# rcallahan/smalt

Measured on AMD Instinct MI355X. Metric: mapped reads/sec (1Mx150bp vs 3Gbp ref), higher is better.
Workload: dtype f16

## Files before the change

### smalt_amd/csrc/smaltgpu.cpp

```cpp
#include <hip/hip_runtime.h>
#include <math.h>
#include <stdarg.h>
#include <stdio.h>
#include <stdlib.h>
#include <string.h>
#include <mutex>
#include <string>
#include <thread>
#include <vector>
#include "../../include/smaltgpu.h"
#include "smg_dump.hpp"
#include "smg_indexfile.hpp"
#include "smg_indexbuild.h"
#include "smg_fasta.hpp"
#include "smg_kernels.h"

using namespace smg;

static thread_local std::string g_err;
static int fail(int code, const char *fmt, ...) {
  char buf[512];
  va_list ap;
  va_start(ap, fmt);
  vsnprintf(buf, sizeof(buf), fmt, ap);
// ... 284 lines not shown
  }
  return ix->packed_host.data();
}

extern "C" int smaltgpu_index_info(const smaltgpu_index *ix, smaltgpu_index_desc *o) {
  if (!ix || !o) return fail(SMALTGPU_EARG, "null argument");
  memset(o, 0, sizeof(*o));
  o->k = ix->d.k; o->s = ix->d.s; o->typ = ix->d.typ; o->nbits_key = ix->d.nbits_key; o->nbits_lo = ix->d.nbits_lo;
  o->npos = ix->d.npos; o->nwords = ix->d.nwords; o->idx = ix->d.idx; o->pos = ix->d.pos; o->wordidx = ix->d.wordidx;
  o->posidx = ix->d.posidx; o->nseq = ix->d.nseq; o->sop = ix->sop.data(); o->packed = ix->d.packed; o->on_device = 1;
  return SMALTGPU_OK;
}

extern "C" void smaltgpu_params_default(smaltgpu_params *p, const smaltgpu_index *ix) {
  memset(p, 0, sizeof(*p));
  p->ktuple_maxhit = 10000;
  p->min_cover = 0;
  p->min_swatscor = ix->d.k + ix->d.s - 1;
  p->min_swatscor_below_max = 0;
  p->min_basqval = 0;
  p->target_depth = 512; p->max_depth = 2048;
  p->rmapflg = SMALTGPU_FLG_BEST | (ix->d.nseq < 512 ? SMALTGPU_FLG_SEQBYSEQ : 0);
  p->match = 1; p->mismatch = -2; p->gap_init = -4; p->gap_ext = -3;
}

enum { T_ENCODE = 0, T_SEED, T_HITS, T_CANDS, T_SW_FULL, T_SW_SCALAR, T_REPLAY, T_ALIGN, T_NUM };
static const char *const kTimerNames[T_NUM] = {"encode", "seed", "hits", "cands", "sw_full", "sw_scalar", "replay", "align"};
extern "C" const char *smaltgpu_timer_name(int i) { return (i >= 0 && i < T_NUM) ? kTimerNames[i] : nullptr; }

struct smaltgpu_mapper {
  const smaltgpu_index *ix = nullptr;
  int device = 0;
  hipStream_t stream = nullptr;
  uint32_t max_reads = 0, max_len = 0, qmax = 0;
  uint64_t max_bases = 0;
  uint8_t *d_bases = nullptr, *d_quals = nullptr, *d_codes = nullptr, *d_codes_rc = nullptr;
  uint64_t *d_off = nullptr;
  uint32_t *d_ids = nullptr;
  uint32_t hits_W = 0, hits_wg = 0;
  HitRun *b_hitrun = nullptr;
  Batch b;
  enum : size_t { CT_LINE = 128, CT_RC = 0, CT_RES = 1 * CT_LINE, CT_DSTR = 2 * CT_LINE, CT_ERR = 3 * CT_LINE, CT_NEXT = 4 * CT_LINE ,
                  CT_ALIGN_RETRY = 9 * CT_LINE, CT_CANDS_RETRY = 10 * CT_LINE, CT_HITS = 11 * CT_LINE, CT_HITS_CURSOR = 12 * CT_LINE, CT_STRIP_CURSOR = 13 * CT_LINE,
                  CT_WORK = 14 * CT_LINE , CT_BYTES = 16 * CT_LINE };
  uint8_t *d_counters = nullptr;
  double *d_logtab = nullptr; uint32_t logtab_n = 0;
  uint8_t *seed_scr = nullptr; size_t seed_bytes = 0; uint32_t seed_slots = 0;
  uint8_t *cand_scr = nullptr; size_t cand_bytes = 0; uint32_t cand_slots = 0;
  CandGeom cg2; uint8_t *cand_scr2 = nullptr; size_t cand_bytes2 = 0; uint32_t cand_slots2 = 0;
  CandGeom cg;
  uint8_t *cand_scr_dbg = nullptr; uint32_t cand_dbg_reads = 0;
  int *sw_rows = nullptr; uint32_t sw_rowlen = 0, sw_threads = 0;
  void *strip_bnd = nullptr; uint8_t *strip_win = nullptr; uint32_t strip_grid = 0;
  uint8_t *align_scr = nullptr; size_t align_bytes = 0; uint32_t align_slots = 0;
  uint8_t *align_scr2 = nullptr; size_t align_bytes2 = 0; uint32_t align_slots2 = 0; uint64_t dircap2 = 0;
  uint32_t wincap = 0, rescap_slot = 0, dstrcap_slot = 0; uint64_t dircap = 0;
  uint32_t rescap_slot2 = 0, dstrcap_slot2 = 0;
  template <class T> struct Pinned {
    T *p = nullptr; size_t cap = 0;
    int ensure(size_t n) {
      if (n <= cap) return 0;
      size_t c = cap ? cap : 1024;
      while (c < n) c += c / 2 + 1;
      T *q = nullptr;
      if (hipHostMalloc((void **)&q, c * sizeof(T), hipHostMallocDefault) != hipSuccess) return -1;
      if (p) (void)hipHostFree(p);
      p = q; cap = c;
      return 0;
    }
    void release() { if (p) (void)hipHostFree(p); p = nullptr; cap = 0; }
    T *data() { return p; }
    T &operator[](size_t i) { return p[i]; }
  };
  Pinned<ReadStat> h_stat;
  Pinned<Result> h_res;
  Pinned<uint8_t> h_dstr;
  hipEvent_t ev_fetch = nullptr;
  uint32_t fetch_n = 0; uint64_t fetch_nres = 0; bool fetch_open = false, pool_overflow = false;
  std::vector<smaltgpu_result> fin_res; std::vector<uint8_t> fin_dstr; std::vector<smaltgpu_readstat> fin_stat; std::vector<uint64_t> fin_off;
  std::vector<uint64_t> h_res_off;
  std::vector<smaltgpu_result> o_res;
  std::vector<smaltgpu_readstat> o_stat;
  std::vector<uint64_t> h_off;
  uint32_t last_n = 0;
  MapPar last_par;
  bool have_host_off = false;
  int debug = 0;
  struct DevBuf {
    void *p = nullptr; size_t cap = 0;
    int ensure(size_t n) { if (n <= cap) return 0; if (p) (void)hipFree(p); p = nullptr; cap = 0; size_t c = n + n / 2 + 256; if (hipMalloc(&p, c) != hipSuccess) return -1; cap = c; return 0; }
    void release() { if (p) (void)hipFree(p); p = nullptr; cap = 0; }
  };
  DevBuf cx_ivoff, cx_iv, cx_minsw, cx_prevmax, cx_fineidx, cx_finepos, cx_fineoff, cx_alloclen, cx_seedrange;
  int host_threads = 1;
  bool history = false;
  uint32_t hist_longest = 0;
  std::vector<uint32_t> h_alloclen;
  std::vector<uint32_t> h_ivoff, h_fineoff;
  std::vector<HitInfoHdr> h_hi;
  bool last_fine = false;
  uint64_t remap_batches = 0;
  hipEvent_t ev[T_NUM + 1] = {nullptr};
  double ms[T_NUM] = {0};
  unsigned long long work[WK_NWORK] = {0};
};

// ... 123 lines not shown
      const size_t fixed = 64  + seqb + (size_t)5 * m->cg.tab * 4 + 64 + 15 + 256 ;
      uint32_t w = fixed + 23 * 256 < 20480 ? (uint32_t)((20480 - fixed) / 23) & ~7u : 256u;
      if (w < (uint32_t)CANDS_LDS_HITS / 2) w = CANDS_LDS_HITS;
      const char *e = getenv("SMALTGPU_CANDS_LDS_HITS");
      m->cg.lds_hits = e ? (uint32_t)atoi(e) : w;
    }
    if (m->cg.lds_hits < 256) m->cg.lds_hits = 256;
    if (m->cg.lds_hits > 2048) m->cg.lds_hits = 2048;
    m->cg.slot_bytes = m->cand_bytes = cand_slot_bytes(m->cg, m->qmax, d.s);
    memset(&m->cg2, 0, sizeof(m->cg2));
    auto geom_for = [&](uint64_t hs) { CandGeom g = m->cg; g.hcap_strand = (uint32_t)hs; g.hcap = (uint32_t)(2 * hs); g.segcap = (uint32_t)hs; g.candcap = (uint32_t)(2 * hs);
                                       g.slot_bytes = cand_slot_bytes(g, m->qmax, d.s); return g; };
    const CandGeom full = m->cg;
    if (m->cand_bytes > (64ull << 20)) {
      uint64_t hs = next_pow2((uint64_t)24 * m->qmax);
      if (const char *e = getenv("SMALTGPU_CANDS_HCAP")) { const long v = atol(e); if (v >= 1024) hs = next_pow2((uint64_t)v); }
      if (hs < m->cg.hcap_strand) { m->cg = geom_for(hs); m->cand_bytes = m->cg.slot_bytes; }
    } else if (const char *e = getenv("SMALTGPU_CANDS_HCAP")) {
      const long v = atol(e);
      if (v >= 1024 && next_pow2((uint64_t)v) < m->cg.hcap_strand) { m->cg = geom_for(next_pow2((uint64_t)v)); m->cand_bytes = m->cg.slot_bytes; }
    }
    {
      uint64_t hw = next_pow2((uint64_t)m->cg.ngrp * alloc);
      if (hw < full.hcap_strand) hw = full.hcap_strand;
      if (hw < (2ull << 20)) hw = 2ull << 20;
      while (hw > full.hcap_strand && (hw > (1ull << 30) || geom_for(hw).slot_bytes > (4ull << 30))) hw >>= 1;
      if (hw > m->cg.hcap_strand) {
        m->cg2 = geom_for(hw); m->cg2.pass = 2; m->cand_bytes2 = m->cg2.slot_bytes;
        m->cg.pass = 1;
        uint64_t n2 = (opt_budget ? ((uint64_t)opt_budget << 30) / 4 : (8ull << 30)) / m->cand_bytes2;
        if (n2 > 8) n2 = 8;
        if (n2 < 1) n2 = 1;
        if (n2 > max_batch_reads) n2 = max_batch_reads;
        m->cand_slots2 = (uint32_t)n2;
        DA(m->cand_scr2, m->cand_bytes2 * m->cand_slots2);
      }
    }
    uint64_t budget = 64ull << 30;
    if (opt_budget) budget = (uint64_t)opt_budget << 30;
    if (const char *e = getenv("SMALTGPU_SLOT_BUDGET_GB")) { const long g = atol(e); if (g > 0) budget = (uint64_t)g << 30; }
    uint64_t slots = budget / m->cand_bytes;
    if (slots > 2048) slots = 2048;
    if (slots < 64) slots = 64;
    if (slots > max_batch_reads) slots = max_batch_reads;
    m->cand_slots = (uint32_t)slots;
    DA(m->cand_scr, m->cand_bytes * m->cand_slots);
  }
  m->sw_rowlen = m->qmax + 8; m->sw_threads = 16384;
  DA(m->sw_rows, (size_t)m->sw_threads * 2 * m->sw_rowlen);
  {
    m->wincap = 4 * m->qmax + 1024;
    m->strip_grid = 5120;
    if (const char *e = getenv("SMALTGPU_STRIP_GRID")) { const long v = atol(e); if (v >= 64 && v <= 16384) m->strip_grid = (uint32_t)v; }
    if ((uint64_t)m->strip_grid * m->wincap * 18 > (8ull << 30)) m->strip_grid = (uint32_t)((8ull << 30) / ((uint64_t)m->wincap * 18));
    if (!rv) rv = dalloc((uint8_t **)&m->strip_bnd, (size_t)m->strip_grid * 2 * m->wincap * 8);
    DA(m->strip_win, (size_t)m->strip_grid * m->wincap * 2);
    m->dircap = (uint64_t)(m->qmax + 64) * (m->wincap + 8);
    m->rescap_slot = 512; m->dstrcap_slot = 512 * (m->qmax / 4 + 48);
    m->rescap_slot2 = 2 * MAXIMUM_DEPTH; m->dstrcap_slot2 = m->rescap_slot2 * (m->qmax / 4 + 48);
    m->dircap2 = m->dircap;
    if (m->dircap > (4ull << 20)) {
      m->dircap2 = m->dircap;
      m->dircap = m->dircap / 16 > (4ull << 20) ? m->dircap / 16 : (4ull << 20);
      if (const char *e = getenv("SMALTGPU_ALIGN_DIRCAP")) { const long v = atol(e); if (v >= 4096 && (uint64_t)v < m->dircap2) m->dircap = (uint64_t)v; }
    }
    m->align_bytes2 = align_scratch_bytes(m->qmax, m->wincap, m->dircap2, m->rescap_slot2, m->dstrcap_slot2);
    m->align_slots2 = max_batch_reads < 16 ? max_batch_reads : 16;
    DA(m->align_scr2, m->align_bytes2 * m->align_slots2);
    m->align_bytes = align_scratch_bytes(m->qmax, m->wincap, m->dircap, m->rescap_slot, m->dstrcap_slot);
    uint64_t budget = 8ull << 30;
    if (m->align_bytes * 512 > budget) budget = m->align_bytes * 512;
    if (budget > (48ull << 30)) budget = 48ull << 30;
    if (opt_budget && ((uint64_t)opt_budget << 30) < budget) budget = (uint64_t)opt_budget << 30;
    if (const char *e = getenv("SMALTGPU_SLOT_BUDGET_GB")) { const uint64_t g = (uint64_t)atol(e) << 30; if (g > 0 && g < budget) budget = g; }
    uint64_t slots = budget / m->align_bytes;
    if (slots > 8192) slots = 8192;
    if (slots < 16) slots = 16;
    if (slots > max_batch_reads) slots = max_batch_reads;
    m->align_slots = (uint32_t)slots;
    DA(m->align_scr, m->align_bytes * m->align_slots);
  }
#undef DA
  if (rv) { smaltgpu_mapper_free(m); return rv; }
  *out = m;
  return SMALTGPU_OK;
}

extern "C" void smaltgpu_mapper_free(smaltgpu_mapper *m) {
  if (!m) return;
  (void)hipSetDevice(m->device);
  void *ps[] = {m->d_bases, m->d_quals, m->d_codes, m->d_codes_rc, m->d_off, m->d_ids, m->b.hi, m->b.seeds, m->b.qmask, m->b.ch, m->b.ctl,
                m->b.stat, m->b.align_retry, m->b.cands_retry, m->d_logtab, m->b.hitpool, m->b_hitrun, m->b.rcpool, m->b.long_list, m->b.strip_list, m->strip_bnd, m->strip_win, m->b.respool, m->b.dstrpool, m->d_counters, m->seed_scr, m->cand_scr, m->cand_scr2, m->cand_scr_dbg,
                m->sw_rows, m->align_scr, m->align_scr2};
  for (void *p : ps) if (p) (void)hipFree(p);
  m->h_stat.release(); m->h_res.release(); m->h_dstr.release();
  m->cx_ivoff.release(); m->cx_iv.release(); m->cx_minsw.release(); m->cx_prevmax.release(); m->cx_fineidx.release(); m->cx_finepos.release(); m->cx_fineoff.release(); m->cx_alloclen.release(); m->cx_seedrange.release();
  if (m->ev_fetch) (void)hipEventDestroy(m->ev_fetch);
  for (int i = 0; i <= T_NUM; i++) if (m->ev[i]) (void)hipEventDestroy(m->ev[i]);
  if (m->stream) (void)hipStreamDestroy(m->stream);
  delete m;
}

extern "C" int smaltgpu_set_debug(smaltgpu_mapper *m, int level) {
  if (!m) return fail(SMALTGPU_EARG, "null mapper");
  m->debug = level;
  return SMALTGPU_OK;
// ... 23 lines not shown
                        const smaltgpu_params *par, const CtxDev *cx = nullptr, bool seed_only = false) {
  Batch &b = m->b;
  const DevIndex &d = m->ix->d;
  MapPar p = to_par(par);
  b.iv_off = cx ? cx->iv_off : nullptr; b.iv = cx ? cx->iv : nullptr; b.min_sw = cx ? cx->min_sw : nullptr; b.prevmax = cx ? cx->prevmax : nullptr;
  b.fine_idx = cx ? cx->fine_idx : nullptr; b.fine_pos = cx ? cx->fine_pos : nullptr; b.fine_off = cx ? cx->fine_off : nullptr;
  b.alloc_len = cx ? cx->alloc_len : nullptr;
  b.seed_range = cx ? cx->seed_range : nullptr;
  b.totals_only = seed_only ? 1u : 0u;
  b.raw_results = cx ? cx->raw : 0u;
  if (b.fine_idx) p.flags |= FLG_NOSHRTINFO;
  m->last_fine = b.fine_idx != nullptr;
  m->last_par = p; m->last_n = n;
  b.nreads = n; b.codes = m->d_codes; b.codes_rc = m->d_codes_rc; b.qual = d_quals; b.read_off = d_off;
  hipStream_t s = m->stream;
  HIPCHK(hipMemsetAsync(m->d_counters, 0, smaltgpu_mapper::CT_BYTES, s));
  int rv = 0;
  const bool seqbyseq = (p.flags & FLG_SEQBYSEQ) != 0;
  const uint32_t ngrp = seqbyseq ? (uint32_t)d.nseq : 1u;
  uint8_t *cscr = m->cand_scr;
  uint32_t cslots = m->cand_slots;
  int slot_per_read = 0;
  CandGeom cgeom = m->cg;
  const bool two_pass = m->cand_scr2 != nullptr && !m->debug;
  const size_t cbytes_dbg = m->cand_bytes;
  if (m->debug) {
    if (n > 2048) return fail(SMALTGPU_EARG, "debug batches are limited to 2048 reads");
    if (m->cand_dbg_reads < n) {
      if (m->cand_scr_dbg) (void)hipFree(m->cand_scr_dbg);
      m->cand_scr_dbg = nullptr;
      HIPCHK(hipMalloc((void **)&m->cand_scr_dbg, cbytes_dbg * n));
      m->cand_dbg_reads = n;
    }
    cscr = m->cand_scr_dbg; cslots = n; slot_per_read = 1;
  }
  HIPCHK(hipEventRecord(m->ev[T_ENCODE], s));
  rv = launch_encode(s, d_bases, d_off, n, m->d_codes, m->d_codes_rc);
  if (!rv && b.fine_idx) rv = launch_fine_index(s, b, d);
  HIPCHK(hipEventRecord(m->ev[T_SEED], s));
  if (!rv) rv = launch_seed(s, b, d, p, m->seed_scr, m->seed_bytes, m->seed_slots);
  HIPCHK(hipEventRecord(m->ev[T_HITS], s));
  const bool split_hits = m->hits_W && m->b_hitrun && !b.iv_off && !seed_only;
  b.hitrun = split_hits ? m->b_hitrun : nullptr;
  if (!rv && split_hits) rv = launch_hits(s, b, d, p, m->hits_W, m->cg.tab, m->hits_wg);
  HIPCHK(hipEventRecord(m->ev[T_CANDS], s));
  if (seed_only) {
    for (int i = T_CANDS + 1; i <= T_NUM; i++) HIPCHK(hipEventRecord(m->ev[i], s));
    if (rv) return fail(SMALTGPU_ENODEV, "kernel launch failed: %s", hipGetErrorString((hipError_t)rv));
    return SMALTGPU_OK;
  }
  { CandGeom g = cgeom; g.ngrp = ngrp; g.debug = slot_per_read; if (!two_pass) g.pass = 0; if (!rv) rv = launch_cands(s, b, d, p, cscr, cslots, g); }
  if (two_pass) { CandGeom g = m->cg2; g.ngrp = ngrp; g.debug = 0; g.pass = 2; if (!rv) rv = launch_cands(s, b, d, p, m->cand_scr2, m->cand_slots2, g); }
  HIPCHK(hipEventRecord(m->ev[T_SW_FULL], s));
  if (!rv) rv = launch_sw_full(s, b, d, p, m->max_len, b.rccap, 8192);
  HIPCHK(hipEventRecord(m->ev[T_SW_SCALAR], s));
  if (!rv) rv = launch_sw_strip(s, b, d, p, m->strip_bnd, m->strip_win, m->wincap, m->strip_grid);
  if (!rv) rv = launch_sw_scalar(s, b, d, p, m->sw_rows, m->sw_rowlen, m->sw_threads, m->max_len);
  HIPCHK(hipEventRecord(m->ev[T_REPLAY], s));
  if (!rv) rv = launch_replay(s, b, d, p);
  HIPCHK(hipEventRecord(m->ev[T_ALIGN], s));
  CplxPar cplx;
  cplx.logtab = m->d_logtab; cplx.nlog = m->logtab_n; cplx.pad = 0;
  cplx.lambda = (p.flags & FLG_CMPLXW) ? cplx_lambda(p.match, p.mismatch) : 0.0;
  if (!rv) rv = launch_align(s, b, d, p, m->align_scr, m->align_bytes, m->align_slots, m->wincap, m->dircap, m->rescap_slot, m->dstrcap_slot, 1, &cplx);
  if (!rv) rv = launch_align(s, b, d, p, m->align_scr2, m->align_bytes2, m->align_slots2, m->wincap, m->dircap2, m->rescap_slot2, m->dstrcap_slot2, 2, &cplx);
  HIPCHK(hipEventRecord(m->ev[T_NUM], s));
  if (rv) return fail(SMALTGPU_ENODEV, "kernel launch failed: %s", hipGetErrorString((hipError_t)rv));
  return SMALTGPU_OK;
}

extern "C" int smaltgpu_synchronize(smaltgpu_mapper *m) {
  if (!m) return fail(SMALTGPU_EARG, "null mapper");
  HIPCHK(hipStreamSynchronize(m->stream));
  return SMALTGPU_OK;
}

extern "C" int smaltgpu_map_batch_device(smaltgpu_mapper *m, const uint8_t *d_bases, const uint8_t *d_quals, const uint64_t *d_read_off,
                                          uint32_t nreads, uint64_t total_bases, const smaltgpu_params *par) {
  if (!m || !d_bases || !d_read_off || !par) return fail(SMALTGPU_EARG, "null argument");
  if (nreads > m->max_reads || total_bases > m->max_bases) return fail(SMALTGPU_EARG, "batch exceeds the mapper's capacity");
  int rv = check_par(m, par);
  if (rv) return rv;
  HIPCHK(hipSetDevice(m->device));
  m->have_host_off = false;
  return run_pipeline(m, d_bases, d_quals, d_read_off, nreads, par);
}

extern "C" int smaltgpu_fetch_begin(smaltgpu_mapper *m) {
  if (!m) return fail(SMALTGPU_EARG, "null argument");
  HIPCHK(hipSetDevice(m->device));
  const uint32_t n = m->last_n;
  uint8_t ctr[smaltgpu_mapper::CT_BYTES];
  if (!m->ev_fetch) HIPCHK(hipEventCreate(&m->ev_fetch));
  if (m->h_stat.ensure(n ? n : 1)) return fail(SMALTGPU_ENOMEM, "pinned host memory");
  HIPCHK(hipMemcpyAsync(ctr, m->d_counters, smaltgpu_mapper::CT_BYTES, hipMemcpyDeviceToHost, m->stream));
  HIPCHK(hipStreamSynchronize(m->stream));
  const uint32_t rc_count = *(uint32_t *)(ctr + smaltgpu_mapper::CT_RC);
  const uint64_t nres = *(unsigned long long *)(ctr + smaltgpu_mapper::CT_RES), ndstr = *(unsigned long long *)(ctr + smaltgpu_mapper::CT_DSTR);
  memcpy(m->work, ctr + smaltgpu_mapper::CT_WORK, sizeof(m->work));
  for (int i = 0; i < T_NUM; i++) { float f = 0; (void)hipEventElapsedTime(&f, m->ev[i], m->ev[i + 1]); m->ms[i] = f; }
  m->fetch_open = false;
  m->pool_overflow = rc_count > m->b.rccap || nres > m->b.rescap || ndstr > m->b.dstrcap;
  const uint64_t nres_c = nres < m->b.rescap ? nres : m->b.rescap, ndstr_c = ndstr < m->b.dstrcap ? ndstr : m->b.dstrcap;
  if (m->h_res.ensure(nres_c ? nres_c : 1) || m->h_dstr.ensure(ndstr_c ? ndstr_c : 1)) return fail(SMALTGPU_ENOMEM, "pinned host memory");
  if (n) HIPCHK(hipMemcpyAsync(m->h_stat.data(), m->b.stat, (size_t)n * sizeof(ReadStat), hipMemcpyDeviceToHost, m->stream));
  if (nres_c) HIPCHK(hipMemcpyAsync(m->h_res.data(), m->b.respool, nres_c * sizeof(Result), hipMemcpyDeviceToHost, m->stream));
  if (ndstr_c) HIPCHK(hipMemcpyAsync(m->h_dstr.data(), m->b.dstrpool, ndstr_c, hipMemcpyDeviceToHost, m->stream));
// ... 485 lines not shown
```

### smalt_amd/csrc/smg_kernels.hip

```cpp
#include <hip/hip_runtime.h>
#include <cstdlib>
#include "smg_kernels.h"
#include "smg_stages.hpp"

namespace smg {

__device__ inline uint8_t code_of(uint8_t c) {
  c &= 0xDF;
  return c == 'A' ? 0 : c == 'C' ? 1 : c == 'G' ? 2 : (c == 'T' || c == 'U') ? 3 : 5;
}

__global__ void __launch_bounds__(64) k_encode(const uint8_t *bases, const uint64_t *off, uint32_t n, uint8_t *codes, uint8_t *codes_rc) {
  for (uint32_t r = blockIdx.x; r < n; r += gridDim.x) {
    const uint64_t o = off[r];
    const uint32_t len = (uint32_t)(off[r + 1] - o);
    for (uint32_t i = threadIdx.x; i < len; i += 64) {
      uint8_t c = code_of(bases[o + i]);
      codes[o + i] = c;
      codes_rc[o + len - 1 - i] = (c & 4) ? c : (uint8_t)(3 - c);
    }
  }
}

__global__ void __launch_bounds__(64) k_gather_reads(uint8_t *dst_bases, uint8_t *dst_quals, const uint64_t *dst_off, uint32_t n, const uint32_t *ids,
// ... 394 lines not shown
#pragma unroll
    for (int c0 = 0; c0 < C; c0 += SW16_BLK) {
      hf2 t3[SW16_BLK];
      const hf2 last_old = H[(c0 + SW16_BLK - 1 < C) ? c0 + SW16_BLK - 1 : C - 1];
#pragma unroll
      for (int u = 0; u < SW16_BLK; u++) {
        const int cc = c0 + u;
        if (cc < C) {
          const hf2 w = __builtin_bit_cast(hf2, __builtin_amdgcn_perm(rr.y, rr.x, sel[cc]));
          const hf2 dg = u == 0 ? carry : H[cc - 1];
          t3[u] = dg + w;
        }
      }
#pragma unroll
      for (int u = 0; u < SW16_BLK; u++) {
        const int cc = c0 + u;
        if (cc < C) {
          const hf2 hh = hf_max3(t3[u], E[cc], F);
          H[cc] = hh;
          const hf2 tt = hh + ngi;
          E[cc] = hf_max3(E[cc] + nge, tt, zero);
          F = hf_max3(F + nge, tt, zero);
        }
      }
#pragma unroll
      for (int u = 0; u < SW16_BLK; u += 2) {
        const int cc = c0 + u;
        if (cc + 1 < C && u + 1 < SW16_BLK) best = hf_max3(best, H[cc], H[cc + 1]);
        else if (cc < C) best = __builtin_elementwise_maximum(best, H[cc]);
      }
      carry = last_old;
    }
  }
  for (int o = G / 2; o > 0; o >>= 1)
    best = __builtin_elementwise_maximum(best, __builtin_bit_cast(hf2, (uint32_t)__shfl_xor((int)__builtin_bit_cast(uint32_t, best), o)));
  return (uint32_t)(int)(float)best.x | ((uint32_t)(int)(float)best.y << 16);
}

__device__ inline void sw16_rowtab(uint32_t *rowtab, const Sw16Par &sp) {
  if (threadIdx.x < 8) rowtab[threadIdx.x] = threadIdx.x < 4 ? sp.mm4 + (sp.dlt << (8 * threadIdx.x)) : sp.n4;
}
__device__ inline void sw16_rowtab2(uint2 *rowtab2, const Sw16Par &sp) {
  const uint32_t a = threadIdx.x & 7u, bq = threadIdx.x >> 3;
  if (sp.fp) {
    const uint32_t x4 = sp.hi_mismatch * 0x01010101u;
    rowtab2[threadIdx.x] = make_uint2(a < 4 ? (x4 & ~(0xffu << (8 * a))) | (sp.hi_match << (8 * a)) : 0u,
                                      bq < 4 ? (x4 & ~(0xffu << (8 * bq))) | (sp.hi_match << (8 * bq)) : 0u);
    return;
  }
  rowtab2[threadIdx.x] = make_uint2(a < 4 ? sp.mm4 + (sp.dlt << (8 * a)) : sp.n4, bq < 4 ? sp.mm4 + (sp.dlt << (8 * bq)) : sp.n4);
}
enum : uint32_t { SW16_NPAIR = 5u | (5u << 3) };

template <int G, int C, int WMAX>
__global__ void __launch_bounds__(64) k_sw_full16(Batch b, DevIndex ix, MapPar p, uint32_t ntask_cap) {
  const unsigned long long nlong = WMAX > SW_SHORT_WMAX ? b.work[WK_LONG_TASKS] : 0;
  if (WMAX > SW_SHORT_WMAX && nlong == 0) return;
  const uint32_t *list = (WMAX > SW_SHORT_WMAX && b.long_list && nlong <= b.long_cap) ? b.long_list : nullptr;
  constexpr int NG = 64 / G;
  __shared__ uint16_t win[NG][WMAX + 2 * G];
  __shared__ uint2 rowtab2[64];
  const int lane = threadIdx.x, g = lane % G, grp = lane / G;
  const uint32_t ntask = list ? (uint32_t)nlong : min(*b.rc_count, ntask_cap), npair = (ntask + 1) / 2;
  const Sw16Par sp = sw16_par(p, G * C);
  sw16_rowtab2(rowtab2, sp);
  const uint32_t ngroups = gridDim.x * NG;
  unsigned long long cells = 0, ntasks_done = 0;
  for (uint32_t t0 = blockIdx.x * NG; t0 < npair; t0 += ngroups) {
    const uint32_t tp = t0 + grp;
    RCand c[2];
    bool live[2] = {false, false};
    uint32_t qlen[2] = {0, 0}, wlen[2] = {0, 0}, tix[2] = {0, 0};
    uint64_t gbase[2] = {0, 0};
    const uint8_t *q[2] = {b.codes, b.codes};
#pragma unroll
    for (int u = 0; u < 2; u++) {
      const uint32_t tl = 2 * tp + (uint32_t)u;
      if (tp < npair && tl < ntask) {
        tix[u] = list ? list[tl] : tl;
        c[u] = b.rcpool[tix[u]];
        qlen[u] = read_len(b, c[u].rid);
        wlen[u] = (uint32_t)(c[u].re - c[u].rs + 1);
        live[u] = !(c[u].flags & (RCF_BANDED | RCF_ERR | RCF_QN | RCF_SCORED)) && wlen[u] <= (uint32_t)WMAX && qlen[u] <= (uint32_t)(G * C);
        gbase[u] = (c[u].sqidx < 0 ? 0ull : ix.sop[c[u].sqidx]) + c[u].rs;
        q[u] = ((c[u].flags & RCF_REVERSE) ? b.codes_rc : b.codes) + b.read_off[c[u].rid];
      }
      if (!live[u]) { qlen[u] = 0; wlen[u] = 0; }
    }
    const uint32_t wmax = wlen[0] > wlen[1] ? wlen[0] : wlen[1];
    int nstep = (int)wmax + G - 1;
    for (int o = 32; o > 0; o >>= 1) nstep = max(nstep, __shfl_xor(nstep, o));
    nstep = __builtin_amdgcn_readfirstlane(nstep);
    {
      const uint32_t nent = (uint32_t)(nstep + G - 1), per = (nent + G - 1) / G;
      const uint32_t e0 = (uint32_t)g * per, e1 = e0 + per < nent ? e0 + per : nent;
      const uint64_t lastw = ix.totlen / 10;
      uint64_t wi[2] = {0, 0};
      uint32_t wd[2] = {0, 0}, nx[2] = {0, 0}, off[2] = {0, 0};
#pragma unroll
      for (int u = 0; u < 2; u++) {
        const int i0 = (int)e0 - (G - 1);
        const uint64_t pos = gbase[u] + (uint64_t)(i0 > 0 ? i0 : 0);
        wi[u] = pos / 10; off[u] = (uint32_t)(pos - wi[u] * 10);
        if (wlen[u] && e0 < e1) { wd[u] = ix.packed[wi[u] < lastw ? wi[u] : lastw]; nx[u] = ix.packed[wi[u] + 1 < lastw ? wi[u] + 1 : lastw]; }
      }
      for (uint32_t e = e0; e < e1; e++) {
        const uint32_t i = e - (uint32_t)(G - 1);
        uint32_t cd[2];
#pragma unroll
        for (int u = 0; u < 2; u++) {
          cd[u] = 5u;
          if (i < wlen[u]) {
            const uint32_t c = (wd[u] >> (3 * (9 - off[u]))) & 7u;
            cd[u] = (c == 7) ? 0u : ((c == 6 || c == 4) ? 5u : c);
            if (++off[u] == 10) { off[u] = 0; wi[u]++; wd[u] = nx[u]; nx[u] = ix.packed[wi[u] + 1 < lastw ? wi[u] + 1 : lastw]; }
          }
        }
        win[grp][e] = (uint16_t)(cd[0] | (cd[1] << 3));
      }
    }
    uint32_t sel[C];
#pragma unroll
    for (int cc = 0; cc < C; cc++) {
      const uint32_t j = (uint32_t)(g * C + cc);
      const uint32_t sa = j < qlen[0] ? (uint32_t)q[0][j] : 0x0cu, sb = j < qlen[1] ? 4u + (uint32_t)q[1][j] : 0x0cu;
      sel[cc] = sp.fp ? (0x000c000cu | (sa << 8) | (sb << 24)) : (0x0c000c00u | sa | (sb << 16));
    }
    __syncthreads();
    const uint32_t bb = sp.fp ? sw16f_core<G, C>(win[grp], nstep, sel, g, sp, rowtab2) : sw16_core<G, C>(win[grp], nstep, sel, g, sp, rowtab2);
    if (g == 0) {
#pragma unroll
      for (int u = 0; u < 2; u++) {
        if (live[u]) {
          const int best = (int)((bb >> (16 * u)) & 0xffffu);
          const uint32_t t = tix[u];
          b.rcpool[t].swscor = best;
          b.rcpool[t].flags = c[u].flags | RCF_SCORED | (best >= 65535 ? RCF_BANDED : 0u);
          cells += (unsigned long long)qlen[u] * wlen[u];
          ntasks_done += best < 65535 ? 1 : 0;
        }
      }
    }
    __syncthreads();
  }
  for (int o = 32; o > 0; o >>= 1) { cells += __shfl_xor(cells, o); ntasks_done += __shfl_xor(ntasks_done, o); }
  if (lane == 0 && cells) { atomicAdd(b.work + WK_CELLS_FULL, cells); atomicAdd(b.work + WK_TASKS_FULL, ntasks_done); }
}

template <int G, int C>
__global__ void __launch_bounds__(64) k_sw_full16_raw(const uint8_t *qcodes, const uint32_t *q_off, const uint8_t *rcodes,
                                                       const uint32_t *r_off, uint32_t ntask, MapPar p, int32_t *scores) {
  constexpr int NG = 64 / G;
  constexpr int WMAX = SW_FULL_WMAX;
  __shared__ uint16_t win[NG][WMAX + 2 * G];
  __shared__ uint2 rowtab2[64];
  const int lane = threadIdx.x, g = lane % G, grp = lane / G;
  const uint32_t npair = (ntask + 1) / 2;
  const Sw16Par sp = sw16_par(p, G * C);
  sw16_rowtab2(rowtab2, sp);
  const uint32_t ngroups = gridDim.x * NG;
  for (uint32_t t0 = blockIdx.x * NG; t0 < npair; t0 += ngroups) {
    const uint32_t tp = t0 + grp;
    bool live[2] = {false, false};
    uint32_t qlen[2] = {0, 0}, wlen[2] = {0, 0};
    const uint8_t *q[2] = {qcodes, qcodes}, *r[2] = {rcodes, rcodes};
#pragma unroll
    for (int u = 0; u < 2; u++) {
      const uint32_t t = 2 * tp + (uint32_t)u;
      if (tp < npair && t < ntask) {
        qlen[u] = q_off[t + 1] - q_off[t]; wlen[u] = r_off[t + 1] - r_off[t];
        q[u] += q_off[t]; r[u] += r_off[t];
        live[u] = wlen[u] <= (uint32_t)WMAX && qlen[u] <= (uint32_t)(G * C);
      }
      if (!live[u]) { qlen[u] = 0; wlen[u] = 0; }
    }
    const uint32_t wmax = wlen[0] > wlen[1] ? wlen[0] : wlen[1];
    int nstep = (int)wmax + G - 1;
    for (int o = 32; o > 0; o >>= 1) nstep = max(nstep, __shfl_xor(nstep, o));
    nstep = __builtin_amdgcn_readfirstlane(nstep);
    for (uint32_t e = g; e < (uint32_t)(nstep + G - 1); e += G) {
      const uint32_t i = e - (uint32_t)(G - 1);
      uint32_t cd[2];
#pragma unroll
      for (int u = 0; u < 2; u++) { const uint32_t x = i < wlen[u] ? (r[u][i] & 7u) : 5u; cd[u] = x == 7 ? 0 : ((x == 6 || x == 4) ? 5 : x); }
      win[grp][e] = (uint16_t)(cd[0] | (cd[1] << 3));
    }
    uint32_t sel[C];
    bool qn[2] = {false, false};
#pragma unroll
    for (int cc = 0; cc < C; cc++) {
      const uint32_t j = (uint32_t)(g * C + cc);
      uint32_t s2[2];
#pragma unroll
      for (int u = 0; u < 2; u++) {
        const uint32_t qc = j < qlen[u] ? (q[u][j] & 7u) : 0x0cu;
        if (j < qlen[u] && qc >= 4) qn[u] = true;
        s2[u] = qc == 0x0cu ? 0x0cu : (uint32_t)(4 * u) + (qc & 3u);
      }
      sel[cc] = sp.fp ? (0x000c000cu | (s2[0] << 8) | (s2[1] << 24)) : (0x0c000c00u | s2[0] | (s2[1] << 16));
    }
#pragma unroll
    for (int u = 0; u < 2; u++) for (int o = G / 2; o > 0; o >>= 1) { const int other = __shfl_xor((int)qn[u], o); qn[u] = qn[u] || other != 0; }
    __syncthreads();
    const uint32_t bb = sp.fp ? sw16f_core<G, C>(win[grp], nstep, sel, g, sp, rowtab2) : sw16_core<G, C>(win[grp], nstep, sel, g, sp, rowtab2);
    if (g == 0) {
#pragma unroll
      for (int u = 0; u < 2; u++) {
        const uint32_t t = 2 * tp + (uint32_t)u;
        if (tp < npair && t < ntask) scores[t] = !live[u] ? -1 : (qn[u] ? -2 : (int)((bb >> (16 * u)) & 0xffffu));
      }
    }
    __syncthreads();
  }
}

enum : int { SW_STRIP_C = 16 };

__device__ inline int sw_strip_core(const uint8_t *q, uint32_t qlen, const uint8_t *win, uint32_t wlen, int2 *bnd, uint32_t wcap,
                                    const uint2 *tab, int2 *ring , int bias, int gi, int ge) {
  constexpr int C = SW_STRIP_C;
  const int g = (int)threadIdx.x;
  int2 *ring_in = ring, *ring_out = ring + 128;
  int best = 0;
  const uint32_t nstrip = (qlen + 64 * C - 1) / (64 * C);
  const int nstep = (int)wlen + 63;
  for (uint32_t sidx = 0; sidx < nstrip; sidx++) {
    const int2 *bprev = bnd + (size_t)((sidx + 1) & 1) * wcap;
    int2 *bnext = bnd + (size_t)(sidx & 1) * wcap;
    uint32_t sel[C];
#pragma unroll
    for (int cc = 0; cc < C; cc++) {
      const uint32_t j = sidx * 64 * C + (uint32_t)(g * C + cc);
      sel[cc] = 0x0c0c0c00u | (j < qlen ? (uint32_t)(q[j] & 7) : 5u);
    }
    int H[C], E[C];
#pragma unroll
    for (int cc = 0; cc < C; cc++) { H[cc] = 0; E[cc] = 0; }
    int F = 0, prev_hl = 0;
    __syncthreads();
    if (sidx > 0) {
      const int r0 = g;
      ring_in[g] = r0 < (int)wlen ? bprev[r0] : make_int2(0, 0);
    }
    __syncthreads();
    for (int step = 0; step < nstep; step++) {
      const int row = step - g;
      if (sidx > 0 && (step & 63) == 0) {
        const int r1 = step + 64 + g;
        ring_in[((step >> 6) + 1) % 2 * 64 + g] = r1 < (int)wlen ? bprev[r1] : make_int2(0, 0);
      }
      const uint32_t rb = (row >= 0 && row < (int)wlen) ? win[row] : 5u;
      const uint2 tr = tab[rb];
      int hl = wave_shr1(H[C - 1]);
      int fin = wave_shr1(F);
      if (g == 0) {
// ... 687 lines not shown
```

Baseline: 772,700.

## Stage query codes in LDS per read and vectorize reference window unpacking

Reworks the full 16-bit SW kernel's data loading. Query codes for each read are staged once into shared memory and shared by all candidates of that read, then fetched as packed 32-bit words and turned into selectors with byte-permute instead of per-byte global loads. The reference window is decoded ten bases per packed word with bit tricks rather than a serial per-base loop, and candidate metadata is loaded by two lanes and broadcast by shuffles instead of every lane reading the whole struct. The full-kernel grid size can now be set from the environment. The cost is extra block-wide barriers and a serialized staging loop when a wavefront holds many distinct reads.

```diff
diff --git a/smalt_amd/csrc/smaltgpu.cpp b/smalt_amd/csrc/smaltgpu.cpp
--- a/smalt_amd/csrc/smaltgpu.cpp
+++ b/smalt_amd/csrc/smaltgpu.cpp
@@ -360,6 +360,7 @@
   uint8_t *cand_scr_dbg = nullptr; uint32_t cand_dbg_reads = 0;
   int *sw_rows = nullptr; uint32_t sw_rowlen = 0, sw_threads = 0;
   void *strip_bnd = nullptr; uint8_t *strip_win = nullptr; uint32_t strip_grid = 0;
+  uint32_t full_grid = 8192;
   uint8_t *align_scr = nullptr; size_t align_bytes = 0; uint32_t align_slots = 0;
   uint8_t *align_scr2 = nullptr; size_t align_bytes2 = 0; uint32_t align_slots2 = 0; uint64_t dircap2 = 0;
   uint32_t wincap = 0, rescap_slot = 0, dstrcap_slot = 0; uint64_t dircap = 0;
@@ -589,6 +590,7 @@
     m->wincap = 4 * m->qmax + 1024;
     m->strip_grid = 5120;
     if (const char *e = getenv("SMALTGPU_STRIP_GRID")) { const long v = atol(e); if (v >= 64 && v <= 16384) m->strip_grid = (uint32_t)v; }
+    if (const char *e = getenv("SMALTGPU_SWFULL_GRID")) { const long v = atol(e); if (v >= 1 && v <= 16384) m->full_grid = (uint32_t)v; }
     if ((uint64_t)m->strip_grid * m->wincap * 18 > (8ull << 30)) m->strip_grid = (uint32_t)((8ull << 30) / ((uint64_t)m->wincap * 18));
     if (!rv) rv = dalloc((uint8_t **)&m->strip_bnd, (size_t)m->strip_grid * 2 * m->wincap * 8);
     DA(m->strip_win, (size_t)m->strip_grid * m->wincap * 2);
@@ -718,7 +720,7 @@
   { CandGeom g = cgeom; g.ngrp = ngrp; g.debug = slot_per_read; if (!two_pass) g.pass = 0; if (!rv) rv = launch_cands(s, b, d, p, cscr, cslots, g); }
   if (two_pass) { CandGeom g = m->cg2; g.ngrp = ngrp; g.debug = 0; g.pass = 2; if (!rv) rv = launch_cands(s, b, d, p, m->cand_scr2, m->cand_slots2, g); }
   HIPCHK(hipEventRecord(m->ev[T_SW_FULL], s));
-  if (!rv) rv = launch_sw_full(s, b, d, p, m->max_len, b.rccap, 8192);
+  if (!rv) rv = launch_sw_full(s, b, d, p, m->max_len, b.rccap, m->full_grid);
   HIPCHK(hipEventRecord(m->ev[T_SW_SCALAR], s));
   if (!rv) rv = launch_sw_strip(s, b, d, p, m->strip_bnd, m->strip_win, m->wincap, m->strip_grid);
   if (!rv) rv = launch_sw_scalar(s, b, d, p, m->sw_rows, m->sw_rowlen, m->sw_threads, m->max_len);
diff --git a/smalt_amd/csrc/smg_kernels.hip b/smalt_amd/csrc/smg_kernels.hip
--- a/smalt_amd/csrc/smg_kernels.hip
+++ b/smalt_amd/csrc/smg_kernels.hip
@@ -470,94 +470,194 @@
 }
 enum : uint32_t { SW16_NPAIR = 5u | (5u << 3) };
 
+template <int G, int C>
+struct Sw16Geo {
+  enum : int { CP = (C + 3) & ~3,
+               NW = CP / 4, QST = G * CP };
+};
+typedef uint32_t __attribute__((may_alias)) u32_alias;
+enum : uint32_t { SW16_PAD4 = 0x0c0c0c0cu, SW16_N10 = 0x2DB6DB6Du  };
+constexpr int sw16_went(int G, int WMAX) { return (WMAX + 2 * G - 2 + 9) / 10 * 10; }
+
+template <int G, int C, bool RAW>
+__device__ inline bool sw16_stage(uint8_t *qst, const uint8_t *fw, const uint8_t *rc, uint32_t qlen) {
+  constexpr uint32_t CP = Sw16Geo<G, C>::CP, QST = Sw16Geo<G, C>::QST;
+  bool bad = false;
+  for (uint32_t t = threadIdx.x; t < QST; t += 64) {
+    const uint32_t gg = t / CP, cc = t % CP, j = gg * (uint32_t)C + cc;
+    uint32_t a = 0x0cu, r = 0x0cu;
+    if (cc < (uint32_t)C && j < qlen) {
+      a = fw[j];
+      if (RAW) { bad = bad || (a & 7u) >= 4u; a &= 3u; r = a; }
+      else r = rc[j];
+    }
+    qst[t] = (uint8_t)a; qst[QST + t] = (uint8_t)r;
+  }
+  return RAW && __any(bad);
+}
+template <int G, int C, int NW>
+__device__ inline void sw16_fetch(uint32_t (&x)[NW], const uint8_t *qst, int g, bool rev) {
+  const u32_alias *src = (const u32_alias *)(qst + (rev ? (int)Sw16Geo<G, C>::QST : 0) + g * (int)Sw16Geo<G, C>::CP);
+#pragma unroll
+  for (int w = 0; w < NW; w++) x[w] = src[w];
+}
+template <int G, int C, int NW>
+__device__ inline void sw16_sel(uint32_t (&sel)[C], const uint32_t (&xa)[NW], const uint32_t (&xb)[NW], int fp) {
+  uint32_t xh[NW];
+#pragma unroll
+  for (int w = 0; w < NW; w++) xh[w] = xb[w] + 0x04040404u - ((xb[w] & 0x08080808u) >> 1);
+  if (fp) {
+#pragma unroll
+    for (int cc = 0; cc < C; cc++) {
+      const uint32_t t = (uint32_t)(cc & 3);
+      sel[cc] = __builtin_amdgcn_perm(xh[cc >> 2], xa[cc >> 2], 0x000c000cu | (t << 8) | ((4u + t) << 24)) | 0x000c000cu;
+    }
+  } else {
+#pragma unroll
+    for (int cc = 0; cc < C; cc++) {
+      const uint32_t t = (uint32_t)(cc & 3);
+      sel[cc] = __builtin_amdgcn_perm(xh[cc >> 2], xa[cc >> 2], 0x0c000c00u | t | ((4u + t) << 16)) | 0x0c000c00u;
+    }
+  }
+}
+
+template <int G>
+__device__ inline void sw16_win_origin(uint64_t gbase, bool small, int64_t &wbase, uint32_t &s) {
+  uint64_t w0; uint32_t r0;
+  if (small) { const uint32_t p32 = (uint32_t)gbase, w = p32 / 10u; w0 = w; r0 = p32 - w * 10u; }
+  else { w0 = gbase / 10; r0 = (uint32_t)(gbase - w0 * 10); }
+  const uint32_t a = r0 + 20u - (uint32_t)(G - 1), qq = a / 10u;
+  s = a - qq * 10u;
+  wbase = (int64_t)w0 - 2 + (int64_t)qq;
+}
+__device__ inline uint32_t sw16_map10(uint32_t w) {
+  const uint32_t b2 = w & 0x24924924u;
+  const uint32_t is7 = b2 & (w << 1) & (w << 2);
+  const uint32_t isn = b2 ^ is7;
+  const uint32_t full = b2 | (b2 >> 1) | (b2 >> 2);
+  return (w & ~full) | isn | (isn >> 2);
+}
+template <int G>
+__device__ inline uint32_t sw16_codes10(const uint32_t *packed, int64_t wbase, uint32_t s, uint32_t m, uint32_t mlo, uint32_t mhi, uint32_t wlen) {
+  const uint32_t ka = min(max(m, mlo), mhi), kb = min(max(m + 1u, mlo), mhi);
+  const uint32_t *pw = packed + wbase;
+  const uint32_t hi = pw[ka] & 0x3fffffffu, lo = pw[kb] & 0x3fffffffu;
+  const uint64_t cat = ((uint64_t)hi << 30) | lo;
+  const uint32_t raw = (uint32_t)(cat >> (3u * (10u - s))) & 0x3fffffffu;
+  const int i0 = (int)(10u * m) - (G - 1);
+  int dlo = -i0, dhi = (int)wlen - i0;
+  dlo = dlo < 0 ? 0 : (dlo > 10 ? 10 : dlo);
+  dhi = dhi < 0 ? 0 : (dhi > 10 ? 10 : dhi);
+  const uint32_t valid = ((1u << (3 * (10 - dlo))) - 1u) & ~((1u << (3 * (10 - dhi))) - 1u);
+  return (sw16_map10(raw) & valid) | (SW16_N10 & ~valid);
+}
+template <int G>
+__device__ inline void sw16_window(uint16_t *wrow, int g, uint32_t nent, const uint32_t *packed, int64_t lastw, const int64_t (&wbase)[2],
+                                   const uint32_t (&ws)[2], const uint32_t (&wlen)[2]) {
+  u32_alias *dst = (u32_alias *)wrow;
+  const uint32_t nchunk = (nent + 9u) / 10u;
+  uint32_t mlo[2], mhi[2];
+#pragma unroll
+  for (int u = 0; u < 2; u++) {
+    const int64_t room = lastw - wbase[u];
+    mlo[u] = wbase[u] < 0 ? (uint32_t)(-wbase[u]) : 0u;
+    mhi[u] = room > 0x7fffffff ? 0x7fffffffu : (uint32_t)room;
+  }
+  for (uint32_t m = (uint32_t)g; m < nchunk; m += G) {
+    const uint32_t ma = sw16_codes10<G>(packed, wbase[0], ws[0], m, mlo[0], mhi[0], wlen[0]);
+    const uint32_t mb = sw16_codes10<G>(packed, wbase[1], ws[1], m, mlo[1], mhi[1], wlen[1]);
+#pragma unroll
+    for (int pr = 0; pr < 5; pr++) {
+      const int s0 = 3 * (9 - 2 * pr), s1 = s0 - 3;
+      const uint32_t e0 = ((ma >> s0) & 7u) | (((mb >> s0) & 7u) << 3), e1 = ((ma >> s1) & 7u) | (((mb >> s1) & 7u) << 3);
+      dst[5 * m + (uint32_t)pr] = e0 | (e1 << 16);
+    }
+  }
+}
+
 template <int G, int C, int WMAX>
 __global__ void __launch_bounds__(64) k_sw_full16(Batch b, DevIndex ix, MapPar p, uint32_t ntask_cap) {
   const unsigned long long nlong = WMAX > SW_SHORT_WMAX ? b.work[WK_LONG_TASKS] : 0;
   if (WMAX > SW_SHORT_WMAX && nlong == 0) return;
   const uint32_t *list = (WMAX > SW_SHORT_WMAX && b.long_list && nlong <= b.long_cap) ? b.long_list : nullptr;
-  constexpr int NG = 64 / G;
-  __shared__ uint16_t win[NG][WMAX + 2 * G];
+  constexpr int NG = 64 / G, NW = Sw16Geo<G, C>::NW;
+  __shared__ __attribute__((aligned(16))) uint16_t win[NG][sw16_went(G, WMAX)];
   __shared__ uint2 rowtab2[64];
+  __shared__ __attribute__((aligned(16))) uint8_t qst[2 * Sw16Geo<G, C>::QST];
   const int lane = threadIdx.x, g = lane % G, grp = lane / G;
   const uint32_t ntask = list ? (uint32_t)nlong : min(*b.rc_count, ntask_cap), npair = (ntask + 1) / 2;
   const Sw16Par sp = sw16_par(p, G * C);
   sw16_rowtab2(rowtab2, sp);
-  const uint32_t ngroups = gridDim.x * NG;
+  const uint32_t niter = (npair + NG - 1) / NG;
+  const bool small = ix.totlen <= 0xffffffffull;
+  const int64_t lastw = (int64_t)(ix.totlen / 10);
+  uint32_t staged = 0xffffffffu;
   unsigned long long cells = 0, ntasks_done = 0;
-  for (uint32_t t0 = blockIdx.x * NG; t0 < npair; t0 += ngroups) {
-    const uint32_t tp = t0 + grp;
-    RCand c[2];
-    bool live[2] = {false, false};
-    uint32_t qlen[2] = {0, 0}, wlen[2] = {0, 0}, tix[2] = {0, 0};
-    uint64_t gbase[2] = {0, 0};
-    const uint8_t *q[2] = {b.codes, b.codes};
+  for (uint32_t it = blockIdx.x; it < niter; it += gridDim.x) {
+    const uint32_t tp = it * NG + grp;
+    uint32_t tix = 0, flags = 0, rid = 0, meta = 0, wlo = 0, whi = 0;
+    {
+      const uint32_t tl = 2 * tp + (uint32_t)g;
+      if (g < 2 && tp < npair && tl < ntask) {
+        tix = list ? list[tl] : tl;
+        const RCand *rc = b.rcpool + tix;
+        flags = rc->flags;
+        const uint32_t r = rc->rid;
+        const uint64_t rs = rc->rs;
+        const uint32_t ql = read_len(b, r), wl = (uint32_t)(rc->re - rs + 1);
+        if (!(flags & (RCF_BANDED | RCF_ERR | RCF_QN | RCF_SCORED)) && wl <= (uint32_t)WMAX && ql <= (uint32_t)(G * C)) {
+          const int32_t sq = rc->sqidx;
+          int64_t wb; uint32_t s;
+          sw16_win_origin<G>((sq < 0 ? 0ull : ix.sop[sq]) + rs, small, wb, s);
+          rid = r; wlo = (uint32_t)(uint64_t)wb; whi = (uint32_t)((uint64_t)wb >> 32);
+          meta = ql | (wl << 10) | (s << 20) | ((flags & RCF_REVERSE) ? 1u << 24 : 0u) | (1u << 25);
+        }
+      }
+    }
+    uint32_t qlen[2], wlen[2], ws[2], key[2];
+    int64_t wbase[2];
+    bool live[2], rev[2];
 #pragma unroll
     for (int u = 0; u < 2; u++) {
-      const uint32_t tl = 2 * tp + (uint32_t)u;
-      if (tp < npair && tl < ntask) {
-        tix[u] = list ? list[tl] : tl;
-        c[u] = b.rcpool[tix[u]];
-        qlen[u] = read_len(b, c[u].rid);
-        wlen[u] = (uint32_t)(c[u].re - c[u].rs + 1);
-        live[u] = !(c[u].flags & (RCF_BANDED | RCF_ERR | RCF_QN | RCF_SCORED)) && wlen[u] <= (uint32_t)WMAX && qlen[u] <= (uint32_t)(G * C);
-        gbase[u] = (c[u].sqidx < 0 ? 0ull : ix.sop[c[u].sqidx]) + c[u].rs;
-        q[u] = ((c[u].flags & RCF_REVERSE) ? b.codes_rc : b.codes) + b.read_off[c[u].rid];
-      }
-      if (!live[u]) { qlen[u] = 0; wlen[u] = 0; }
+      const int src = (lane & ~(G - 1)) + u;
+      const uint32_t mt = (uint32_t)__shfl((int)meta, src);
+      key[u] = (uint32_t)__shfl((int)rid, src);
+      wbase[u] = (int64_t)(((uint64_t)(uint32_t)__shfl((int)whi, src) << 32) | (uint32_t)__shfl((int)wlo, src));
+      qlen[u] = mt & 0x3ffu; wlen[u] = (mt >> 10) & 0x3ffu; ws[u] = (mt >> 20) & 0xfu; rev[u] = (mt >> 24) & 1u; live[u] = (mt >> 25) & 1u;
     }
     const uint32_t wmax = wlen[0] > wlen[1] ? wlen[0] : wlen[1];
     int nstep = (int)wmax + G - 1;
     for (int o = 32; o > 0; o >>= 1) nstep = max(nstep, __shfl_xor(nstep, o));
     nstep = __builtin_amdgcn_readfirstlane(nstep);
-    {
-      const uint32_t nent = (uint32_t)(nstep + G - 1), per = (nent + G - 1) / G;
-      const uint32_t e0 = (uint32_t)g * per, e1 = e0 + per < nent ? e0 + per : nent;
-      const uint64_t lastw = ix.totlen / 10;
-      uint64_t wi[2] = {0, 0};
-      uint32_t wd[2] = {0, 0}, nx[2] = {0, 0}, off[2] = {0, 0};
-#pragma unroll
-      for (int u = 0; u < 2; u++) {
-        const int i0 = (int)e0 - (G - 1);
-        const uint64_t pos = gbase[u] + (uint64_t)(i0 > 0 ? i0 : 0);
-        wi[u] = pos / 10; off[u] = (uint32_t)(pos - wi[u] * 10);
-        if (wlen[u] && e0 < e1) { wd[u] = ix.packed[wi[u] < lastw ? wi[u] : lastw]; nx[u] = ix.packed[wi[u] + 1 < lastw ? wi[u] + 1 : lastw]; }
-      }
-      for (uint32_t e = e0; e < e1; e++) {
-        const uint32_t i = e - (uint32_t)(G - 1);
-        uint32_t cd[2];
-#pragma unroll
-        for (int u = 0; u < 2; u++) {
-          cd[u] = 5u;
-          if (i < wlen[u]) {
-            const uint32_t c = (wd[u] >> (3 * (9 - off[u]))) & 7u;
-            cd[u] = (c == 7) ? 0u : ((c == 6 || c == 4) ? 5u : c);
-            if (++off[u] == 10) { off[u] = 0; wi[u]++; wd[u] = nx[u]; nx[u] = ix.packed[wi[u] + 1 < lastw ? wi[u] + 1 : lastw]; }
-          }
-        }
-        win[grp][e] = (uint16_t)(cd[0] | (cd[1] << 3));
-      }
+    sw16_window<G>(win[grp], g, (uint32_t)(nstep + G - 1), ix.packed, lastw, wbase, ws, wlen);
+    uint32_t xa[NW], xb[NW];
+#pragma unroll
+    for (int w = 0; w < NW; w++) { xa[w] = SW16_PAD4; xb[w] = SW16_PAD4; }
+    bool pend0 = live[0], pend1 = live[1];
+    for (;;) {
+      const unsigned long long pm = __ballot(pend0 || pend1);
+      if (!pm) break;
+      const uint32_t R = (uint32_t)__builtin_amdgcn_readlane((int)(pend0 ? key[0] : key[1]), __ffsll(pm) - 1);
+      if (R != staged) {
+        __syncthreads();
+        const uint64_t o = b.read_off[R];
+        sw16_stage<G, C, false>(qst, b.codes + o, b.codes_rc + o, (uint32_t)(b.read_off[R + 1] - o));
+        staged = R;
+        __syncthreads();
+      }
+      if (pend0 && key[0] == R) { sw16_fetch<G, C>(xa, qst, g, rev[0]); pend0 = false; }
+      if (pend1 && key[1] == R) { sw16_fetch<G, C>(xb, qst, g, rev[1]); pend1 = false; }
     }
     uint32_t sel[C];
-#pragma unroll
-    for (int cc = 0; cc < C; cc++) {
-      const uint32_t j = (uint32_t)(g * C + cc);
-      const uint32_t sa = j < qlen[0] ? (uint32_t)q[0][j] : 0x0cu, sb = j < qlen[1] ? 4u + (uint32_t)q[1][j] : 0x0cu;
-      sel[cc] = sp.fp ? (0x000c000cu | (sa << 8) | (sb << 24)) : (0x0c000c00u | sa | (sb << 16));
-    }
+    sw16_sel<G, C>(sel, xa, xb, sp.fp);
     __syncthreads();
     const uint32_t bb = sp.fp ? sw16f_core<G, C>(win[grp], nstep, sel, g, sp, rowtab2) : sw16_core<G, C>(win[grp], nstep, sel, g, sp, rowtab2);
-    if (g == 0) {
-#pragma unroll
-      for (int u = 0; u < 2; u++) {
-        if (live[u]) {
-          const int best = (int)((bb >> (16 * u)) & 0xffffu);
-          const uint32_t t = tix[u];
-          b.rcpool[t].swscor = best;
-          b.rcpool[t].flags = c[u].flags | RCF_SCORED | (best >= 65535 ? RCF_BANDED : 0u);
-          cells += (unsigned long long)qlen[u] * wlen[u];
-          ntasks_done += best < 65535 ? 1 : 0;
-        }
-      }
+    if ((meta >> 25) & 1u) {
+      const int best = (int)((bb >> (16 * g)) & 0xffffu);
+      b.rcpool[tix].swscor = best;
+      b.rcpool[tix].flags = flags | RCF_SCORED | (best >= 65535 ? RCF_BANDED : 0u);
+      cells += (unsigned long long)(meta & 0x3ffu) * ((meta >> 10) & 0x3ffu);
+      ntasks_done += best < 65535 ? 1 : 0;
     }
     __syncthreads();
   }
@@ -568,10 +668,11 @@
 template <int G, int C>
 __global__ void __launch_bounds__(64) k_sw_full16_raw(const uint8_t *qcodes, const uint32_t *q_off, const uint8_t *rcodes,
                                                        const uint32_t *r_off, uint32_t ntask, MapPar p, int32_t *scores) {
-  constexpr int NG = 64 / G;
+  constexpr int NG = 64 / G, NW = Sw16Geo<G, C>::NW;
   constexpr int WMAX = SW_FULL_WMAX;
   __shared__ uint16_t win[NG][WMAX + 2 * G];
   __shared__ uint2 rowtab2[64];
+  __shared__ __attribute__((aligned(16))) uint8_t qst[2 * Sw16Geo<G, C>::QST];
   const int lane = threadIdx.x, g = lane % G, grp = lane / G;
   const uint32_t npair = (ntask + 1) / 2;
   const Sw16Par sp = sw16_par(p, G * C);
@@ -580,14 +681,14 @@
   for (uint32_t t0 = blockIdx.x * NG; t0 < npair; t0 += ngroups) {
     const uint32_t tp = t0 + grp;
     bool live[2] = {false, false};
-    uint32_t qlen[2] = {0, 0}, wlen[2] = {0, 0};
-    const uint8_t *q[2] = {qcodes, qcodes}, *r[2] = {rcodes, rcodes};
+    uint32_t qlen[2] = {0, 0}, wlen[2] = {0, 0}, key[2] = {0, 0};
+    const uint8_t *r[2] = {rcodes, rcodes};
 #pragma unroll
     for (int u = 0; u < 2; u++) {
       const uint32_t t = 2 * tp + (uint32_t)u;
       if (tp < npair && t < ntask) {
         qlen[u] = q_off[t + 1] - q_off[t]; wlen[u] = r_off[t + 1] - r_off[t];
-        q[u] += q_off[t]; r[u] += r_off[t];
+        r[u] += r_off[t]; key[u] = t;
         live[u] = wlen[u] <= (uint32_t)WMAX && qlen[u] <= (uint32_t)(G * C);
       }
       if (!live[u]) { qlen[u] = 0; wlen[u] = 0; }
@@ -603,22 +704,24 @@
       for (int u = 0; u < 2; u++) { const uint32_t x = i < wlen[u] ? (r[u][i] & 7u) : 5u; cd[u] = x == 7 ? 0 : ((x == 6 || x == 4) ? 5 : x); }
       win[grp][e] = (uint16_t)(cd[0] | (cd[1] << 3));
     }
+    uint32_t xa[NW], xb[NW];
+#pragma unroll
+    for (int w = 0; w < NW; w++) { xa[w] = SW16_PAD4; xb[w] = SW16_PAD4; }
+    bool qn[2] = {false, false};
+    bool pend0 = live[0], pend1 = live[1];
+    for (;;) {
+      const unsigned long long pm = __ballot(pend0 || pend1);
+      if (!pm) break;
+      const uint32_t R = (uint32_t)__builtin_amdgcn_readlane((int)(pend0 ? key[0] : key[1]), __ffsll(pm) - 1);
+      __syncthreads();
+      const uint32_t o = q_off[R];
+      const bool bad = sw16_stage<G, C, true>(qst, qcodes + o, qcodes + o, q_off[R + 1] - o);
+      __syncthreads();
+      if (pend0 && key[0] == R) { sw16_fetch<G, C>(xa, qst, g, false); qn[0] = bad; pend0 = false; }
+      if (pend1 && key[1] == R) { sw16_fetch<G, C>(xb, qst, g, false); qn[1] = bad; pend1 = false; }
+    }
     uint32_t sel[C];
-    bool qn[2] = {false, false};
-#pragma unroll
-    for (int cc = 0; cc < C; cc++) {
-      const uint32_t j = (uint32_t)(g * C + cc);
-      uint32_t s2[2];
-#pragma unroll
-      for (int u = 0; u < 2; u++) {
-        const uint32_t qc = j < qlen[u] ? (q[u][j] & 7u) : 0x0cu;
-        if (j < qlen[u] && qc >= 4) qn[u] = true;
-        s2[u] = qc == 0x0cu ? 0x0cu : (uint32_t)(4 * u) + (qc & 3u);
-      }
-      sel[cc] = sp.fp ? (0x000c000cu | (s2[0] << 8) | (s2[1] << 24)) : (0x0c000c00u | s2[0] | (s2[1] << 16));
-    }
-#pragma unroll
-    for (int u = 0; u < 2; u++) for (int o = G / 2; o > 0; o >>= 1) { const int other = __shfl_xor((int)qn[u], o); qn[u] = qn[u] || other != 0; }
+    sw16_sel<G, C>(sel, xa, xb, sp.fp);
     __syncthreads();
     const uint32_t bb = sp.fp ? sw16f_core<G, C>(win[grp], nstep, sel, g, sp, rowtab2) : sw16_core<G, C>(win[grp], nstep, sel, g, sp, rowtab2);
     if (g == 0) {
```

New measurement: 786,900, median of 6. 1.02x the previous value.
